# jianzhnie/ScaleRL

Measured on NVIDIA H100. Metric: learner_frames_per_sec, higher is better.
Workload: dtype bf16

## Files before the change

### scalerl_b200/csrc/enc_fused.cuh

```cuda
#pragma once
#include "igemm_tma.cuh"
#include "encoder_problems.cuh"

namespace srl {

constexpr int FF_THREADS = 544;
constexpr int FF_CONV_WARPS = 8;
constexpr int FF_W1_BYTES = 4 * 32 * 128;
constexpr int FF_W2_BYTES = 8 * 64 * 128;
constexpr int FF_U8_BYTES = 28 * 1024;
constexpr int FF_X_BYTES = 19 * 1024;
constexpr int FF_A1_PLANE = 13 * 1024;
constexpr int FF_A1_BYTES = 31 * 1024;
constexpr int FF_OFF_W2 = FF_W1_BYTES;
constexpr int FF_OFF_U8 = FF_OFF_W2 + FF_W2_BYTES;
constexpr int FF_OFF_X = FF_OFF_U8 + 2 * FF_U8_BYTES;
constexpr int FF_XS = 2;
constexpr int FF_OFF_A1 = FF_OFF_X + FF_XS * FF_X_BYTES;
constexpr int FF_OFF_IMG = FF_OFF_A1 + FF_A1_BYTES;
constexpr int FF_OFF_BAR = FF_OFF_IMG + WG_IMG_BYTES;
constexpr int FF_SMEM_BYTES = FF_OFF_BAR + 1024 + 1024;
static_assert(FF_SMEM_BYTES <= 232448, "shared memory budget");
static_assert(FF_OFF_U8 % 1024 == 0 && FF_OFF_X % 1024 == 0 && FF_OFF_A1 % 1024 == 0, "swizzle atoms need 1024-byte aligned tiles");

struct EncFusedParams {
  const uint8_t* obs;
  const float* w1;
  const float* b1;
  const float* w2;
  const float* b2;
  bf16* xs;
  bf16* a1;
  bf16* a2;
  int frames;
  int NFS;
};

SRL_DEVINL void mbar_wait_relaxed(uint64_t* bar, uint32_t parity) {
  uint32_t spins = 0;
  while (!mbar_try_wait(bar, parity)) {
    __nanosleep(32);
    if (++spins > SRL_SPIN_LIMIT) __trap();
  }
}
SRL_DEVINL void bulk_load_1d(void* dst, const void* src, uint32_t bytes, uint64_t* bar) {
  asm volatile("cp.async.bulk.shared::cluster.global.mbarrier::complete_tx::bytes [%0], [%1], %2, [%3];"
               ::"r"(smem_u32(dst)), "l"(src), "r"(bytes), "r"(smem_u32(bar)) : "memory");
}

__global__ void __launch_bounds__(FF_THREADS, 1) enc_fused_fwd_kernel(const EncFusedParams p) {
  extern __shared__ uint8_t smem_raw[];
  uint8_t* smem = reinterpret_cast<uint8_t*>((reinterpret_cast<uintptr_t>(smem_raw) + 1023) & ~uintptr_t(1023));
  uint8_t* sW1 = smem;
  uint8_t* sW2 = smem + FF_OFF_W2;
  uint8_t* sU8 = smem + FF_OFF_U8;
  uint8_t* sX = smem + FF_OFF_X;
  uint8_t* sA1 = smem + FF_OFF_A1;
  uint64_t* bars = reinterpret_cast<uint64_t*>(smem + FF_OFF_BAR);
  uint64_t* u8_full = bars;
  uint64_t* u8_empty = bars + 2;
  uint64_t* x_full = bars + 4;
  uint64_t* x_empty = bars + 7;
  uint64_t* a1_full = bars + 18;
  uint64_t* a1_empty = bars + 19;
  float* img = reinterpret_cast<float*>(smem + FF_OFF_IMG);
  const int tid = threadIdx.x, warp = tid >> 5, lane = tid & 31;
  const int nmine = p.frames > (int)blockIdx.x ? (p.frames - (int)blockIdx.x + (int)gridDim.x - 1) / (int)gridDim.x : 0;

  float* s_b1 = reinterpret_cast<float*>(smem + FF_OFF_BAR + 256);
  float* s_b2 = s_b1 + 32;
  if (tid < 32) s_b1[tid] = __ldg(p.b1 + tid);
  else if (tid < 96) s_b2[tid - 32] = __ldg(p.b2 + tid - 32);
  if (warp == 16 && lane == 0) {
    for (int i = 0; i < 2; ++i) { mbar_init(&u8_full[i], 1); mbar_init(&u8_empty[i], FF_CONV_WARPS); }
    for (int i = 0; i < FF_XS; ++i) { mbar_init(&x_full[i], FF_CONV_WARPS); mbar_init(&x_empty[i], 4); }
    mbar_init(a1_full, 4); mbar_init(a1_empty, 4);
    mbar_fence_init();
  }
  for (int i = tid; i < (FF_A1_BYTES - 2 * FF_A1_PLANE) / 16; i += FF_THREADS)
    reinterpret_cast<uint4*>(sA1 + 2 * FF_A1_PLANE)[i] = make_uint4(0, 0, 0, 0);
  pdl_wait(54);
// ... 26 lines not shown
          const int co = q >> 7, c = (q >> 2) & 31, kh = q & 3;
          const float w[4] = {v[u].x, v[u].y, v[u].z, v[u].w};
#pragma unroll
          for (int kw = 0; kw < 4; ++kw) {
            const int j = kh * 2 + (kw >> 1), k = (kw & 1) * 32 + c;
            *reinterpret_cast<__nv_bfloat16*>(sW2 + j * 8192 + swz128(co, k >> 3) + (k & 7) * 2) = __float2bfloat16_rn(w[kw]);
          }
        }
      }
    }
  }
  fence_proxy_async_smem();
  __syncthreads();

  if (warp == 16) {
    if (lane == 0) {
      for (int it = 0; it < nmine; ++it) {
        const int f = blockIdx.x + it * gridDim.x, ub = it & 1;
        mbar_wait(&u8_empty[ub], ((it >> 1) & 1) ^ 1);
        mbar_arrive_expect_tx(&u8_full[ub], 28224);
        bulk_load_1d(sU8 + ub * FF_U8_BYTES, p.obs + (size_t)f * 28224, 28224, &u8_full[ub]);
      }
    }
  } else if (warp >= 8) {
    const int t = tid - 256, gp = t & 7, rb = t >> 3;
    const int src_g = (gp >> 1) * 7056 + (gp & 1) * 168;
    for (int it = 0; it < nmine; ++it) {
      const int f = blockIdx.x + it * gridDim.x, ub = it & 1;
      mbar_wait_relaxed(&u8_full[ub], (it >> 1) & 1);
      const uint8_t* u8 = sU8 + ub * FF_U8_BYTES + src_g;
      bf16* xs_f = p.xs + (size_t)f * 441 * 64 + gp * 8;
      for (int j = 0; j < 4; ++j) {
        const int n = 4 * it + j, s = n % FF_XS;
        uint32_t w0[5], w1[5];
        int Qs[5];
        {
          int Q = j * 128 + rb, Y = Q / 21, X = Q - Y * 21;
#pragma unroll
          for (int k = 0; k < 5; ++k) {
            Qs[k] = Q;
            if (rb + 32 * k < 150 && Q < 441) {
              w0[k] = *reinterpret_cast<const uint32_t*>(u8 + Y * 336 + 4 * X);
              w1[k] = *reinterpret_cast<const uint32_t*>(u8 + Y * 336 + 84 + 4 * X);
            }
            Q += 32; X += 11; Y += 1;
            if (X >= 21) { X -= 21; Y += 1; }
          }
        }
        mbar_wait(&x_empty[s], ((n / FF_XS) & 1) ^ 1);
        uint8_t* x = sX + s * FF_X_BYTES;
#pragma unroll
        for (int k = 0; k < 5; ++k) {
          const int row = rb + 32 * k;
          if (row < 150) {
            uint4 v = make_uint4(0u, 0u, 0u, 0u);
            if (Qs[k] < 441) {
              v = u8x8_to_bf16x8(w0[k], w1[k]);
              if (row < 128) *reinterpret_cast<uint4*>(xs_f + (size_t)Qs[k] * 64) = v;
            }
            *reinterpret_cast<uint4*>(x + swz128(row, gp)) = v;
          }
        }
        fence_proxy_async_smem();
        __syncwarp();
        if (lane == 0) mbar_arrive(&x_full[s]);
      }
      __syncwarp();
      if (lane == 0) mbar_arrive(&u8_empty[ub]);
    }
  } else if (warp < 4) {
    const uint64_t w1d = make_smem_desc(smem_u32(sW1), 16, 1024);
    for (int it = 0; it < nmine; ++it) {
      const int f = blockIdx.x + it * gridDim.x;
      for (int j = 0; j < 4; ++j) {
        const int n = 4 * it + j, s = n % FF_XS;
        mbar_wait(&x_full[s], (n / FF_XS) & 1);
        const uint64_t xd = make_smem_desc(smem_u32(sX + s * FF_X_BYTES), 16, 1024);
        float acc[2][16];
        wg_fence();
#pragma unroll
        for (int tap = 0; tap < 4; ++tap)
#pragma unroll
          for (int k = 0; k < 4; ++k)
            wg_mma128<32, 0, 0>(acc, xd + (uint64_t)(((tap >> 1) * 21 + (tap & 1)) * 8 + k * 2), 64 * 128 / 16, w1d + (uint64_t)(tap * 256 + k * 2),
                                (tap | k) != 0);
        wg_commit();
        wg_wait_all();
        wg_fence_regs(acc[0]); wg_fence_regs(acc[1]);
        __syncwarp();
        if (lane == 0) mbar_arrive(&x_empty[s]);
        float r0[16], r1[16];
        wg_acc_row16<32, true>(acc, 0, img, tid, 2, r0);
        wg_acc_row16<32, true>(acc, 1, img, tid, 2, r1);
        if (j == 0) mbar_wait_relaxed(a1_empty, (it & 1) ^ 1);
        const int Q = j * 128 + tid, oh = Q / 21, ow = Q - oh * 21;
// ... 72 lines not shown
```

### scalerl_b200/csrc/encoder.cu

```cuda
#include "encoder_problems.cuh"
#include "tma_problems.cuh"
#include "res_problems.cuh"
#include "enc_fused.cuh"
#include "kernels.h"
#include <stdio.h>
#include <stdlib.h>

namespace srl {

constexpr int PACK_BLOCKS_FK = 256, PACK_BLOCKS_FD = 256, PACK_BLOCKS_CONV = 288;
SRL_DEVINL void pack_store(bf16* __restrict__ out, bf16* __restrict__ out_lo, int64_t i, float v) {
  const bf16 hi = __float2bfloat16_rn(v);
  out[i] = hi;
  if (out_lo) out_lo[i] = __float2bfloat16_rn(v - __bfloat162float(hi));
}
SRL_DEVINL void pack_store2(bf16* __restrict__ out, bf16* __restrict__ out_lo, int64_t i, float v0, float v1) {
  const bf16 h0 = __float2bfloat16_rn(v0), h1 = __float2bfloat16_rn(v1);
  *reinterpret_cast<uint32_t*>(out + i) = pack_bf16x2(v0, v1);
  if (out_lo) *reinterpret_cast<uint32_t*>(out_lo + i) = pack_bf16x2(v0 - __bfloat162float(h0), v1 - __bfloat162float(h1));
}
__global__ void __launch_bounds__(256) pack_weights_kernel(ParamPtrs p, bf16* __restrict__ out, bf16* __restrict__ out_lo, int skip_w1k) {
  pdl_wait(2);
  __shared__ __align__(16) float tile[64 * 99];
  const int t = threadIdx.x, b = blockIdx.x;
// ... 281 lines not shown
  if (t >= w) return;
  float s = 0.f;
  for (int c = 0; c < n; ++c) s += stage[c * w + t];
  if (bias) db[t] += s;
  else g[(size_t)(co0 + (t & 7)) * (L::ROW_GROUPS * L::NR) + L::NR * rg + (t >> 3)] = L::FRAMES_U8 ? s * (1.0f / 255.0f) : s;
}

template <class L>
static cudaError_t launch_wgrad_reduce(const float* part, int n, float* g, float* db, cudaStream_t st) {
  static PerDeviceOnce once;
  SRL_TRY(ensure_max_dynamic_smem(once, conv_wgrad_reduce_kernel<L>, WG_PART_CTAS * L::NR * 32));
  static const int greatest = [] { int lo = 0, hi = 0; return cudaDeviceGetStreamPriorityRange(&lo, &hi) == cudaSuccess ? hi : 0; }();
  cudaLaunchConfig_t cfg = {};
  cfg.gridDim = dim3(L::ROW_GROUPS * (L::CO / 8) + 1); cfg.blockDim = dim3(L::NR * 8); cfg.dynamicSmemBytes = (size_t)n * L::NR * 32; cfg.stream = st;
  cudaLaunchAttribute attr[1];
  attr[0].id = cudaLaunchAttributePriority;
  attr[0].val.priority = greatest;
  cfg.attrs = attr; cfg.numAttrs = 1;
  return cudaLaunchKernelEx(&cfg, conv_wgrad_reduce_kernel<L>, part, n, g, db);
}

cudaError_t encoder_forward(const uint8_t* obs, int frames, const ParamPtrs& p, const EncoderBuffers& buf, const TmaMaps& maps, int mode,
                            const StepStreams& S, bool fused_front) {
  if (frames <= 0) return cudaSuccess;
  if ((mode != 0 && mode != 1) || !maps.valid) return cudaErrorInvalidValue;
  const int sp = mode;
  if (sp && !buf.lo.wpack) return cudaErrorInvalidValue;
  const cudaStream_t st = S.main;
  if (fused_front && !sp && (reinterpret_cast<uintptr_t>(obs) & 15) == 0) {
    EncFusedParams q{obs, p.w1, p.b1, p.w2, p.b2, buf.xs, buf.hi.a1, buf.hi.a2, frames, buf.NF};
    S.b(PS_ENC_FUSED); SRL_TRY(enc_fused_fwd_launch(q, kPersistentCtas, st)); S.e(PS_ENC_FUSED);
    SRL_TRY(S.join(LANE_PACK));
  } else {
  S.b(PS_S2D); SRL_TRY(launch_s2d(obs, frames, buf.xs, st, p.w1, buf.hi.wpack + WPack::W1K, sp ? buf.lo.wpack + WPack::W1K : nullptr)); S.e(PS_S2D);
  { RConv1Fwd::Params q{maps.xs_w, maps.hi.w1k, maps.lo.w1k, p.b1, buf.hi.a1, buf.lo.a1, frames, buf.NF};
    S.b(PS_CONV1_FWD); SRL_TRY(res_fwd_launch<RConv1Fwd>(q, cdiv(frames * 441, 128), kPersistentCtas, st, sp)); S.e(PS_CONV1_FWD); }
  SRL_TRY(S.join(LANE_PACK));
  { RConv2Fwd::Params q{maps.hi.a1p0_w, maps.hi.a1p1_w, maps.hi.w2k, maps.lo.a1p0_w, maps.lo.a1p1_w, maps.lo.w2k, p.b2, buf.hi.a2, buf.lo.a2, frames};
    S.b(PS_CONV2_FWD); SRL_TRY(res_fwd_launch<RConv2Fwd>(q, cdiv(frames * 100, 128), kPersistentCtas, st, sp)); S.e(PS_CONV2_FWD); }
  }
  { RConv3Fwd::Params q{maps.hi.a2_w, maps.hi.w3k, maps.lo.a2_w, maps.lo.w3k, p.b3, buf.hi.a3, buf.lo.a3, frames};
    S.b(PS_CONV3_FWD); SRL_TRY(res_fwd_launch<RConv3Fwd>(q, cdiv(frames * 81, 128), kPersistentCtas, st, sp)); S.e(PS_CONV3_FWD); }
  { TFcFwd::Params q{maps.hi.a3m128, maps.hi.wfk, maps.lo.a3m128, maps.lo.wfk, buf.hpart, frames};
    static_assert(TFcFwd::SPLITS == FC_SPLITS, "split count");
    S.b(PS_FC_FWD);
    if (sp) SRL_TRY((igemm_tma_launch<TFcFwd, 1>(q, dim3(cdiv(frames, 128), 8 * FC_SPLITS), st)));
    else SRL_TRY((igemm_tma_launch<TFcFwd, 0>(q, dim3(cdiv(frames, 128), 8 * FC_SPLITS), st)));
    S.e(PS_FC_FWD); }
  return cudaSuccess;
}

cudaError_t encoder_backward(int frames, const EncoderBuffers& buf, const ParamPtrs& g, const TmaMaps& maps, int mode,
                             const StepStreams& S, BwdParts parts, bool a3t_done) {
  if (frames <= 0) return cudaSuccess;
  if ((mode != 0 && mode != 1) || !maps.valid) return cudaErrorInvalidValue;
  const int sp = mode;
  if (sp && !buf.lo.wpack) return cudaErrorInvalidValue;
  const bool do_fc = parts & BWD_FC, do_conv = parts & BWD_CONV;
  const cudaStream_t st = S.main, s1 = S.lane(LANE_FC_WGRAD), s2 = S.lane(LANE_CONV3_WGRAD), s3 = S.lane(LANE_CONV2_WGRAD);
  if (do_fc) {
    SRL_TRY(S.fork(LANE_FC_WGRAD));
    { const bool native = !sp && buf.a3t != nullptr;
      S.b(PS_FC_WGRAD);
      if (native) {
        if (!a3t_done) SRL_TRY(launch_a3_transpose(buf.hi.a3, buf.a3t, frames, s1));
        TFcWgradN::Params q{maps.hi.dhm64, maps.a3tm64, g.wf, g.bf, frames};
        SRL_TRY((igemm_tma_launch<TFcWgradN, 0>(q, dim3(1, 4 * (TFcWgradN::NCT + 1)), s1)));
      } else {
        TFcWgrad::Params q{maps.hi.dhm64, maps.hi.a3m64, maps.lo.dhm64, maps.lo.a3m64, g.wf, g.bf, frames};
// ... 43 lines not shown
```

### scalerl_b200/csrc/encoder_problems.cuh

```cuda
#pragma once
#include "common.cuh"

namespace srl {

typedef __nv_bfloat16 bf16;

SRL_DEVINL uint4 ldg16(const void* p) { return __ldg(reinterpret_cast<const uint4*>(p)); }

SRL_DEVINL uint4 u8x8_to_bf16x8(uint32_t w0, uint32_t w1) {
  float f[8];
  f[0] = __uint_as_float(__byte_perm(w0, 0x4B000000u, 0x7540)) - 8388608.f;
  f[1] = __uint_as_float(__byte_perm(w0, 0x4B000000u, 0x7541)) - 8388608.f;
  f[2] = __uint_as_float(__byte_perm(w0, 0x4B000000u, 0x7542)) - 8388608.f;
  f[3] = __uint_as_float(__byte_perm(w0, 0x4B000000u, 0x7543)) - 8388608.f;
  f[4] = __uint_as_float(__byte_perm(w1, 0x4B000000u, 0x7540)) - 8388608.f;
  f[5] = __uint_as_float(__byte_perm(w1, 0x4B000000u, 0x7541)) - 8388608.f;
  f[6] = __uint_as_float(__byte_perm(w1, 0x4B000000u, 0x7542)) - 8388608.f;
  f[7] = __uint_as_float(__byte_perm(w1, 0x4B000000u, 0x7543)) - 8388608.f;
  return make_uint4(pack_bf16x2(f[0], f[1]), pack_bf16x2(f[2], f[3]), pack_bf16x2(f[4], f[5]), pack_bf16x2(f[6], f[7]));
}

SRL_DEVINL void store_bf16x16(bf16* dst, const float (&v)[16]) {
  uint4 a = make_uint4(pack_bf16x2(v[0], v[1]), pack_bf16x2(v[2], v[3]), pack_bf16x2(v[4], v[5]), pack_bf16x2(v[6], v[7]));
  uint4 b = make_uint4(pack_bf16x2(v[8], v[9]), pack_bf16x2(v[10], v[11]), pack_bf16x2(v[12], v[13]), pack_bf16x2(v[14], v[15]));
  reinterpret_cast<uint4*>(dst)[0] = a;
  reinterpret_cast<uint4*>(dst)[1] = b;
}
SRL_DEVINL void relu_mask16(const bf16* mask, float (&v)[16]) {
  uint4 a = ldg16(mask), b = ldg16(mask + 8);
  const uint32_t w[8] = {a.x, a.y, a.z, a.w, b.x, b.y, b.z, b.w};
#pragma unroll
  for (int i = 0; i < 8; ++i) {
    if (!(bf16_lo(w[i]) > 0.f)) v[2 * i] = 0.f;
    if (!(bf16_hi(w[i]) > 0.f)) v[2 * i + 1] = 0.f;
  }
}

SRL_DEVINL void relu_mask16_pre(const uint4 (&m)[2], float (&v)[16]) {
  const uint32_t w[8] = {m[0].x, m[0].y, m[0].z, m[0].w, m[1].x, m[1].y, m[1].z, m[1].w};
#pragma unroll
  for (int i = 0; i < 8; ++i) {
    if (!(bf16_lo(w[i]) > 0.f)) v[2 * i] = 0.f;
    if (!(bf16_hi(w[i]) > 0.f)) v[2 * i + 1] = 0.f;
  }
}
SRL_DEVINL void ld_mask16(const bf16* mask, uint4 (&m)[2]) { m[0] = ldg16(mask); m[1] = ldg16(mask + 8); }
SRL_DEVINL uint32_t relu_mask_bf16x2(uint32_t x, uint32_t m) {
  return (bf16_lo(m) > 0.f ? x & 0xFFFFu : 0u) | (bf16_hi(m) > 0.f ? x & 0xFFFF0000u : 0u);
}

}
```

### scalerl_b200/csrc/igemm_res.cuh

```cuda
#pragma once
#include "igemm_tma.cuh"

namespace srl {

constexpr int RES_THREADS = 384;
constexpr int RES_PRODUCER_REGS = 40, RES_CONSUMER_REGS = 232;
constexpr int RES_MAX_TAPS = 10;


template <int N, int ROWB, class F>
SRL_DEVINL void wg_acc_stage_bf16(const float (&d)[2][N / 2], uint8_t* buf, int wt, int bar, F f) {
  static_assert(ROWB % 16 == 0 && ROWB >= 2 * N, "16-byte aligned rows that hold N bf16");
  const int w = wt >> 5, l = wt & 31;
  named_bar(bar, 128);
#pragma unroll
  for (int h = 0; h < 2; ++h)
#pragma unroll
    for (int i = 0; i < N / 2; i += 2) {
      const int row = 64 * h + 16 * w + (l >> 2) + 8 * ((i >> 1) & 1), col = 8 * (i >> 2) + 2 * (l & 3);
      *reinterpret_cast<uint32_t*>(buf + row * ROWB + col * 2) = pack_bf16x2(f(col, d[h][i]), f(col + 1, d[h][i + 1]));
    }
  named_bar(bar, 128);
}
template <class P, int SPLIT>
struct ResFwdCfg {
  static constexpr int ALO = (SPLIT && P::A_LO) ? 1 : 0;
  static constexpr int WIN_BYTES = ((P::WROWS * 128 + 1023) / 1024) * 1024;
  static constexpr int IN_HI_BYTES = P::NWIN * WIN_BYTES;
  static constexpr int IN_BYTES = IN_HI_BYTES * (1 + ALO);
  static constexpr int W_HI_BYTES = P::NT * P::BN * 128;
  static constexpr int W_BYTES = W_HI_BYTES * (1 + SPLIT);
  static constexpr bool TILE_EPI = P::TILE_ROWB > 0 && !SPLIT;
  static constexpr int TILE_IMG_BYTES = 128 * P::TILE_ROWB > WG_IMG_BYTES ? 128 * P::TILE_ROWB : WG_IMG_BYTES;
  static constexpr bool IMG1 = !TILE_EPI && W_BYTES + IN_BYTES + 2 * WG_IMG_BYTES + 1024 + 256 > 232448;
  static constexpr int IMG_BYTES = TILE_EPI ? TILE_IMG_BYTES : IMG1 ? WG_IMG_BYTES / 2 : WG_IMG_BYTES;
  static constexpr int FIT = fit_stages(SPLIT ? P::SPLIT_STAGES : P::STAGES, W_BYTES + 2 * IMG_BYTES + 1024 + 256, IN_BYTES);
  static constexpr int STAGES = FIT > 1 ? FIT & ~1 : 1;
  static constexpr int SMEM_BYTES = W_BYTES + STAGES * IN_BYTES + 2 * IMG_BYTES + 1024 + 256;
  static_assert(SMEM_BYTES <= 232448, "shared memory budget (227 KB)");
  static_assert(W_BYTES % 1024 == 0, "weight block alignment");
  static_assert(P::BN == 32 || P::BN == 64 || P::BN == 128, "MMA N");
};

template <class P, int SPLIT>
__global__ void __launch_bounds__(RES_THREADS, 1) res_fwd_kernel(const __grid_constant__ typename P::Params p) {
  using C = ResFwdCfg<P, SPLIT>;
  constexpr int STAGES = C::STAGES;
  extern __shared__ uint8_t smem_raw[];
  uint8_t* smem = reinterpret_cast<uint8_t*>((reinterpret_cast<uintptr_t>(smem_raw) + 1023) & ~uintptr_t(1023));
  uint8_t* sW = smem;
  uint8_t* sIn = smem + C::W_BYTES;
  float* img = reinterpret_cast<float*>(sIn + STAGES * C::IN_BYTES);
  uint64_t* bars = reinterpret_cast<uint64_t*>(sIn + STAGES * C::IN_BYTES + 2 * C::IMG_BYTES);
  uint64_t* in_full = bars;
  uint64_t* in_empty = bars + STAGES;
  uint64_t* w_full = bars + 2 * STAGES;
  const int tid = threadIdx.x, warp = tid >> 5;
  const int ntiles = P::num_tiles(p);

  if (warp == 8 && (tid & 31) == 0) {
    for (int s = 0; s < STAGES; ++s) { mbar_init(&in_full[s], 1); mbar_init(&in_empty[s], 4); }
    mbar_init(w_full, 1);
    mbar_fence_init();
    P::prefetch(p);
  }
  __syncthreads();

  if (warp >= 8) {
    reg_release<RES_PRODUCER_REGS>();
    if (warp != 8) return;
    const uint32_t leader = elect_one_sync();
    auto load_weights = [&]() {
      mbar_arrive_expect_tx(w_full, C::W_BYTES);
      for (int j = 0; j < P::NT; ++j) tma_load_2d(sW + j * P::BN * 128, &p.w, w_full, j * 64, 0);
      if constexpr (SPLIT)
        for (int j = 0; j < P::NT; ++j) tma_load_2d(sW + C::W_HI_BYTES + j * P::BN * 128, &p.w_lo, w_full, j * 64, 0);
    };
    if (leader && !P::W_AFTER_WAIT) load_weights();
    __syncwarp();
    pdl_wait();
    if (leader) pdl_launch();
    if (leader && P::W_AFTER_WAIT) load_weights();
    __syncwarp();
    int it = 0;
    for (int t = blockIdx.x; t < ntiles; t += gridDim.x, ++it) {
      const int s = it % STAGES;
      mbar_wait(&in_empty[s], ((it / STAGES) & 1) ^ 1);
      if (leader) {
        mbar_arrive_expect_tx(&in_full[s], P::NWIN * P::WROWS * 128 * (1 + C::ALO));
        P::load_windows(p, t, sIn + s * C::IN_BYTES, C::WIN_BYTES, &in_full[s], false);
        if constexpr (C::ALO) P::load_windows(p, t, sIn + s * C::IN_BYTES + C::IN_HI_BYTES, C::WIN_BYTES, &in_full[s], true);
      }
      __syncwarp();
    }
  } else {
    reg_claim<RES_CONSUMER_REGS>();
    pdl_wait(P::KID);
    const int g = warp >> 2, wt = tid & 127;
    float* my_img = img + g * (C::IMG_BYTES / 4);
    constexpr uint32_t A_HI = 64 * 128 / 16;
    mbar_wait(w_full, 0);
    const uint64_t wd = make_smem_desc(smem_u32(sW), 16, 1024);
    int it = 0;
    for (int t = blockIdx.x; t < ntiles; t += gridDim.x, ++it) {
      if (STAGES > 1 ? (it & 1) != g : g != 0) continue;
      const int s = it % STAGES;
      uint4 pre[P::BN / 16][2];
      if constexpr (C::TILE_EPI) P::prefetch_tile(p, t, wt, pre);
      else {
#pragma unroll
        for (int c = 0; c < P::BN / 16; ++c) P::prefetch16(p, t, wt, c * 16, pre[c]);
      }
      float acc[2][P::BN / 2];
      mbar_wait(&in_full[s], (it / STAGES) & 1);
      const uint64_t ind = make_smem_desc(smem_u32(sIn + s * C::IN_BYTES), 16, 1024);
      wg_fence();
#pragma unroll
      for (int j = 0; j < P::NT; ++j) {
        const uint64_t ad = ind + (uint64_t)((P::tap_win(j) * C::WIN_BYTES + P::tap_shift(j) * 128) / 16);
        const uint64_t bd = wd + (uint64_t)(j * P::BN * 128 / 16);
#pragma unroll
        for (int k = 0; k < 4; ++k) {
          wg_mma128<P::BN, 0, 0>(acc, ad + 2 * k, A_HI, bd + 2 * k, (j | k) != 0);
          if constexpr (SPLIT)
            wg_mma128<P::BN, 0, 0>(acc, ad + 2 * k, A_HI, bd + (uint64_t)(C::W_HI_BYTES / 16 + 2 * k), 1);
          if constexpr (C::ALO)
            wg_mma128<P::BN, 0, 0>(acc, ad + (uint64_t)(C::IN_HI_BYTES / 16 + 2 * k), A_HI, bd + 2 * k, 1);
        }
      }
// ... 279 lines not shown
```

### scalerl_b200/csrc/igemm_tma.cuh

```cuda
#pragma once
#include <cuda.h>
#include "common.cuh"
#include "kernels.h"

namespace srl {

SRL_DEVINL void tma_prefetch_desc(const CUtensorMap* m) {
  asm volatile("prefetch.tensormap [%0];" ::"l"(reinterpret_cast<uint64_t>(m)) : "memory");
}
SRL_DEVINL void tma_load_2d(void* dst, const CUtensorMap* m, uint64_t* bar, int c0, int c1) {
  asm volatile("cp.async.bulk.tensor.2d.shared::cluster.global.mbarrier::complete_tx::bytes [%0], [%1, {%3, %4}], [%2];"
               ::"r"(smem_u32(dst)), "l"(reinterpret_cast<uint64_t>(m)), "r"(smem_u32(bar)), "r"(c0), "r"(c1) : "memory");
}
SRL_DEVINL void tma_load_3d(void* dst, const CUtensorMap* m, uint64_t* bar, int c0, int c1, int c2) {
  asm volatile("cp.async.bulk.tensor.3d.shared::cluster.global.mbarrier::complete_tx::bytes [%0], [%1, {%3, %4, %5}], [%2];"
               ::"r"(smem_u32(dst)), "l"(reinterpret_cast<uint64_t>(m)), "r"(smem_u32(bar)), "r"(c0), "r"(c1), "r"(c2) : "memory");
}
SRL_DEVINL void tma_load_4d(void* dst, const CUtensorMap* m, uint64_t* bar, int c0, int c1, int c2, int c3) {
  asm volatile("cp.async.bulk.tensor.4d.shared::cluster.global.mbarrier::complete_tx::bytes [%0], [%1, {%3, %4, %5, %6}], [%2];"
               ::"r"(smem_u32(dst)), "l"(reinterpret_cast<uint64_t>(m)), "r"(smem_u32(bar)), "r"(c0), "r"(c1), "r"(c2), "r"(c3)
               : "memory");
}
SRL_DEVINL void tma_load_5d(void* dst, const CUtensorMap* m, uint64_t* bar, int c0, int c1, int c2, int c3, int c4) {
  asm volatile("cp.async.bulk.tensor.5d.shared::cluster.global.mbarrier::complete_tx::bytes [%0], [%1, {%3, %4, %5, %6, %7}], [%2];"
               ::"r"(smem_u32(dst)), "l"(reinterpret_cast<uint64_t>(m)), "r"(smem_u32(bar)), "r"(c0), "r"(c1), "r"(c2), "r"(c3), "r"(c4)
               : "memory");
}

constexpr int IGT_THREADS = 288;

template <class P, int SPLIT = 0>
struct TmaCfg {
  static constexpr int KROWS = P::A_MN ? P::KROWS : 64;
  static constexpr int A_BYTES = P::A_MN ? 2 * KROWS * 128 : 128 * 128;
  static constexpr int B_BLOCKS = (P::BN + 63) / 64;
  static constexpr int B_BYTES = P::B_MN ? B_BLOCKS * KROWS * 128 : P::BN * 128;
  static constexpr int HALF_BYTES = A_BYTES + B_BYTES;
  static constexpr int STAGE_BYTES = HALF_BYTES * (1 + SPLIT);
  static constexpr int NB = P::BN / 2;
  static constexpr int STAGES = fit_stages(P::STAGES, 2 * WG_IMG_BYTES + 1024 + 256, STAGE_BYTES);
  static constexpr int SMEM_BYTES = STAGES * STAGE_BYTES + 2 * WG_IMG_BYTES + 1024 + 256;
  static_assert(SMEM_BYTES <= 232448, "shared memory budget (227 KB)");
  static_assert(NB == 32 || NB == 64 || NB == 128, "MMA N per warpgroup");
  static constexpr int MMAS = P::A_MN ? KROWS / 16 : 4;
  static constexpr bool TILE_EPI = P::TILE_ROWB > 0 && !SPLIT;
// ... 149 lines not shown
```

### scalerl_b200/csrc/res_problems.cuh

```cuda
#pragma once
#include "igemm_res.cuh"
#include "encoder_problems.cuh"

namespace srl {

template <int SPLIT>
SRL_DEVINL void store_act16(bf16* hi, bf16* lo, size_t elem_off, const float (&v)[16]) {
  store_bf16x16(hi + elem_off, v);
  if constexpr (SPLIT) {
    float r[16];
#pragma unroll
    for (int j = 0; j < 16; ++j) r[j] = v[j] - __bfloat162float(__float2bfloat16_rn(v[j]));
    store_bf16x16(lo + elem_off, r);
  }
}

struct RConv1Fwd {
  static constexpr int KID = 11;
  static constexpr int BN = 32, NT = 4, NWIN = 1, WROWS = 128 + 22, STAGES = 4, SPLIT_STAGES = 4;
  static constexpr bool A_LO = false;
  struct Params { SRL_TMAP in0; SRL_TMAP w; SRL_TMAP w_lo; const float* bias; bf16* out; bf16* out_lo; int NF; int NFS; };
  static constexpr bool W_AFTER_WAIT = true;
  SRL_DEVINL static void prefetch(const Params& p) { tma_prefetch_desc(&p.in0); tma_prefetch_desc(&p.w); }
  SRL_DEVINL static int num_tiles(const Params& p) { return (p.NF * 441 + 127) >> 7; }
  SRL_DEVINL static constexpr int tap_win(int) { return 0; }
  SRL_DEVINL static constexpr int tap_shift(int j) { return (j >> 1) * 21 + (j & 1); }
  SRL_DEVINL static void load_windows(const Params& p, int t, uint8_t* dst, int, uint64_t* bar, bool) { tma_load_2d(dst, &p.in0, bar, 0, t * 128); }
  SRL_DEVINL static void prefetch16(const Params&, int, int, int, uint4 (&)[2]) {}
  static constexpr int TILE_ROWB = 80;
  SRL_DEVINL static void prefetch_tile(const Params&, int, int, uint4 (&)[BN / 16][2]) {}
  SRL_DEVINL static void epilogue_tile(const Params& p, int t, int wt, const float (&acc)[2][BN / 2], uint8_t* img, int bar,
                                       const uint4 (&)[BN / 16][2]) {
    wg_acc_stage_bf16<BN, TILE_ROWB>(acc, img, wt, bar, [&](int c, float v) { return fmaxf(fmaf(v, 1.0f / 255.0f, __ldg(p.bias + c)), 0.f); });
#pragma unroll
    for (int s = 0; s < 4; ++s) {
      const int e = s * 128 + wt, q = e >> 2, k = e & 3;
      const int Q = t * 128 + q, n = Q / 441, r = Q - n * 441, oh = r / 21, ow = r - oh * 21;
      if (n >= p.NF || oh >= 20 || ow >= 20) continue;
      const size_t prow = (size_t)(oh & 1) * p.NFS * 100 + (size_t)n * 100 + (oh >> 1) * 10 + (ow >> 1);
      *reinterpret_cast<uint4*>(p.out + prow * 64 + (ow & 1) * 32 + k * 8) = *reinterpret_cast<const uint4*>(img + q * TILE_ROWB + k * 16);
    }
  }
  template <int SPLIT>
  SRL_DEVINL static void epilogue16(const Params& p, int t, int row, int c0, float (&v)[16], const uint4 (&)[2]) {
    const int Q = t * 128 + row, n = Q / 441, r = Q - n * 441, oh = r / 21, ow = r - oh * 21;
    if (n >= p.NF || oh >= 20 || ow >= 20) return;
#pragma unroll
    for (int j = 0; j < 16; ++j) v[j] = fmaxf(fmaf(v[j], 1.0f / 255.0f, __ldg(p.bias + c0 + j)), 0.f);
    const size_t prow = (size_t)(oh & 1) * p.NFS * 100 + (size_t)n * 100 + (oh >> 1) * 10 + (ow >> 1);
    store_act16<SPLIT>(p.out, p.out_lo, prow * 64 + (ow & 1) * 32 + c0, v);
  }
};

struct RConv2Fwd {
  static constexpr int KID = 12;
  static constexpr bool W_AFTER_WAIT = false;
  static constexpr int BN = 64, NT = 8, NWIN = 2, WROWS = 128 + 11, STAGES = 3, SPLIT_STAGES = 1;
  static constexpr bool A_LO = true;
  struct Params { SRL_TMAP in0; SRL_TMAP in1; SRL_TMAP w; SRL_TMAP in0_lo; SRL_TMAP in1_lo; SRL_TMAP w_lo; const float* bias; bf16* out; bf16* out_lo; int NF; };
  SRL_DEVINL static void prefetch(const Params& p) { tma_prefetch_desc(&p.in0); tma_prefetch_desc(&p.in1); tma_prefetch_desc(&p.w); }
  SRL_DEVINL static int num_tiles(const Params& p) { return (p.NF * 100 + 127) >> 7; }
  SRL_DEVINL static constexpr int tap_win(int j) { return (j >> 1) & 1; }
  SRL_DEVINL static constexpr int tap_shift(int j) { return (j >> 2) * 10 + (j & 1); }
  SRL_DEVINL static void load_windows(const Params& p, int t, uint8_t* dst, int win_bytes, uint64_t* bar, bool lo) {
    tma_load_2d(dst, lo ? &p.in0_lo : &p.in0, bar, 0, t * 128);
    tma_load_2d(dst + win_bytes, lo ? &p.in1_lo : &p.in1, bar, 0, t * 128);
  }
  SRL_DEVINL static void prefetch16(const Params&, int, int, int, uint4 (&)[2]) {}
  static constexpr int TILE_ROWB = 144;
  SRL_DEVINL static void prefetch_tile(const Params&, int, int, uint4 (&)[BN / 16][2]) {}
  SRL_DEVINL static void epilogue_tile(const Params& p, int t, int wt, const float (&acc)[2][BN / 2], uint8_t* img, int bar,
                                       const uint4 (&)[BN / 16][2]) {
    wg_acc_stage_bf16<BN, TILE_ROWB>(acc, img, wt, bar, [&](int c, float v) { return fmaxf(v + __ldg(p.bias + c), 0.f); });
#pragma unroll
    for (int s = 0; s < 8; ++s) {
      const int e = s * 128 + wt, q = e >> 3, k = e & 7;
      const int Q = t * 128 + q, n = Q / 100, r = Q - n * 100, oh = r / 10, ow = r - oh * 10;
      if (n >= p.NF || oh >= 9 || ow >= 9) continue;
      *reinterpret_cast<uint4*>(p.out + ((size_t)n * 81 + oh * 9 + ow) * 64 + k * 8) = *reinterpret_cast<const uint4*>(img + q * TILE_ROWB + k * 16);
    }
  }
  template <int SPLIT>
  SRL_DEVINL static void epilogue16(const Params& p, int t, int row, int c0, float (&v)[16], const uint4 (&)[2]) {
    const int Q = t * 128 + row, n = Q / 100, r = Q - n * 100, oh = r / 10, ow = r - oh * 10;
    if (n >= p.NF || oh >= 9 || ow >= 9) return;
#pragma unroll
    for (int j = 0; j < 16; ++j) v[j] = fmaxf(v[j] + __ldg(p.bias + c0 + j), 0.f);
    store_act16<SPLIT>(p.out, p.out_lo, ((size_t)n * 81 + oh * 9 + ow) * 64 + c0, v);
  }
};

struct RConv3Fwd {
  static constexpr int KID = 13;
  static constexpr bool W_AFTER_WAIT = false;
  static constexpr int BN = 64, NT = 9, NWIN = 1, WROWS = 128 + 20, STAGES = 4, SPLIT_STAGES = 2;
  static constexpr bool A_LO = true;
  struct Params { SRL_TMAP in0; SRL_TMAP w; SRL_TMAP in0_lo; SRL_TMAP w_lo; const float* bias; bf16* out; bf16* out_lo; int NF; };
  SRL_DEVINL static void prefetch(const Params& p) { tma_prefetch_desc(&p.in0); tma_prefetch_desc(&p.w); }
  SRL_DEVINL static int num_tiles(const Params& p) { return (p.NF * 81 + 127) >> 7; }
  SRL_DEVINL static constexpr int tap_win(int) { return 0; }
  SRL_DEVINL static constexpr int tap_shift(int j) { return (j / 3) * 9 + j % 3; }
  SRL_DEVINL static void load_windows(const Params& p, int t, uint8_t* dst, int, uint64_t* bar, bool lo) { tma_load_2d(dst, lo ? &p.in0_lo : &p.in0, bar, 0, t * 128); }
  SRL_DEVINL static void prefetch16(const Params&, int, int, int, uint4 (&)[2]) {}
  static constexpr int TILE_ROWB = 144;
  SRL_DEVINL static void prefetch_tile(const Params&, int, int, uint4 (&)[BN / 16][2]) {}
  SRL_DEVINL static void epilogue_tile(const Params& p, int t, int wt, const float (&acc)[2][BN / 2], uint8_t* img, int bar,
                                       const uint4 (&)[BN / 16][2]) {
    wg_acc_stage_bf16<BN, TILE_ROWB>(acc, img, wt, bar, [&](int c, float v) { return fmaxf(v + __ldg(p.bias + c), 0.f); });
#pragma unroll
    for (int s = 0; s < 8; ++s) {
      const int e = s * 128 + wt, q = e >> 3, k = e & 7;
      const int Q = t * 128 + q, n = Q / 81, r = Q - n * 81, oh = r / 9, ow = r - oh * 9;
      if (n >= p.NF || oh >= 7 || ow >= 7) continue;
      *reinterpret_cast<uint4*>(p.out + ((size_t)n * 49 + oh * 7 + ow) * 64 + k * 8) = *reinterpret_cast<const uint4*>(img + q * TILE_ROWB + k * 16);
    }
  }
  template <int SPLIT>
  SRL_DEVINL static void epilogue16(const Params& p, int t, int row, int c0, float (&v)[16], const uint4 (&)[2]) {
    const int Q = t * 128 + row, n = Q / 81, r = Q - n * 81, oh = r / 9, ow = r - oh * 9;
    if (n >= p.NF || oh >= 7 || ow >= 7) return;
#pragma unroll
    for (int j = 0; j < 16; ++j) v[j] = fmaxf(v[j] + __ldg(p.bias + c0 + j), 0.f);
    store_act16<SPLIT>(p.out, p.out_lo, ((size_t)n * 49 + oh * 7 + ow) * 64 + c0, v);
  }
};

struct RConv3Dgrad {
  static constexpr int KID = 14;
  static constexpr bool W_AFTER_WAIT = false;
  static constexpr int BN = 64, NT = 9, NWIN = 1, WROWS = 128 + 20, STAGES = 4, SPLIT_STAGES = 2;
  static constexpr bool A_LO = true;
  struct Params { SRL_TMAP in0; SRL_TMAP w; SRL_TMAP in0_lo; SRL_TMAP w_lo; const bf16* act; bf16* dx; bf16* dx_lo; int NB; };
  SRL_DEVINL static void prefetch(const Params& p) { tma_prefetch_desc(&p.in0); tma_prefetch_desc(&p.w); }
  SRL_DEVINL static int num_tiles(const Params& p) { return (p.NB * 81 + 127) >> 7; }
  SRL_DEVINL static constexpr int tap_win(int) { return 0; }
  SRL_DEVINL static constexpr int tap_shift(int j) { return 20 - ((j / 3) * 9 + j % 3); }
  SRL_DEVINL static void load_windows(const Params& p, int t, uint8_t* dst, int, uint64_t* bar, bool lo) { tma_load_2d(dst, lo ? &p.in0_lo : &p.in0, bar, 0, t * 128 - 20); }
  SRL_DEVINL static void prefetch16(const Params& p, int t, int row, int c0, uint4 (&m)[2]) {
    const int Q = t * 128 + row;
    if (Q < p.NB * 81) ld_mask16(p.act + (size_t)Q * 64 + c0, m);
  }
  static constexpr int TILE_ROWB = 144;
  SRL_DEVINL static void prefetch_tile(const Params& p, int t, int wt, uint4 (&m)[BN / 16][2]) {
#pragma unroll
    for (int s = 0; s < 8; ++s) {
      const int e = s * 128 + wt, Q = t * 128 + (e >> 3);
      if (Q < p.NB * 81) m[s >> 1][s & 1] = ldg16(p.act + (size_t)Q * 64 + (e & 7) * 8);
    }
  }
  SRL_DEVINL static void epilogue_tile(const Params& p, int t, int wt, const float (&acc)[2][BN / 2], uint8_t* img, int bar,
                                       const uint4 (&m)[BN / 16][2]) {
    wg_acc_stage_bf16<BN, TILE_ROWB>(acc, img, wt, bar, [](int, float v) { return v; });
#pragma unroll
    for (int s = 0; s < 8; ++s) {
      const int e = s * 128 + wt, q = e >> 3, k = e & 7;
      const int Q = t * 128 + q, n = Q / 81, r = Q - n * 81, ih = r / 9, iw = r - ih * 9;
      if (n >= p.NB) continue;
      const uint4 x = *reinterpret_cast<const uint4*>(img + q * TILE_ROWB + k * 16), mk = m[s >> 1][s & 1];
      *reinterpret_cast<uint4*>(p.dx + ((size_t)n * 100 + ih * 10 + iw) * 64 + k * 8) =
          make_uint4(relu_mask_bf16x2(x.x, mk.x), relu_mask_bf16x2(x.y, mk.y), relu_mask_bf16x2(x.z, mk.z), relu_mask_bf16x2(x.w, mk.w));
    }
  }
  template <int SPLIT>
  SRL_DEVINL static void epilogue16(const Params& p, int t, int row, int c0, float (&v)[16], const uint4 (&m)[2]) {
    const int Q = t * 128 + row, n = Q / 81, r = Q - n * 81, ih = r / 9, iw = r - ih * 9;
    if (n >= p.NB) return;
    relu_mask16_pre(m, v);
    store_act16<SPLIT>(p.dx, p.dx_lo, ((size_t)n * 100 + ih * 10 + iw) * 64 + c0, v);
  }
};

struct RConv2Dgrad {
  static constexpr int KID = 15;
  static constexpr bool W_AFTER_WAIT = false;
  static constexpr int BN = 128, NT = 4, NWIN = 1, WROWS = 128 + 11, STAGES = 3, SPLIT_STAGES = 2;
  static constexpr bool A_LO = true;
  struct Params { SRL_TMAP in0; SRL_TMAP w; SRL_TMAP in0_lo; SRL_TMAP w_lo; const bf16* act; bf16* dx; bf16* dx_lo; int NB; int NF; };
  SRL_DEVINL static void prefetch(const Params& p) { tma_prefetch_desc(&p.in0); tma_prefetch_desc(&p.w); }
  SRL_DEVINL static int num_tiles(const Params& p) { return (p.NB * 100 + 127) >> 7; }
  SRL_DEVINL static constexpr int tap_win(int) { return 0; }
  SRL_DEVINL static constexpr int tap_shift(int j) { return 11 - ((j >> 1) * 10 + (j & 1)); }
  SRL_DEVINL static void load_windows(const Params& p, int t, uint8_t* dst, int, uint64_t* bar, bool lo) { tma_load_2d(dst, lo ? &p.in0_lo : &p.in0, bar, 0, t * 128 - 11); }
  SRL_DEVINL static void prefetch16(const Params& p, int t, int row, int c0, uint4 (&m)[2]) {
    const int Q = t * 128 + row, cls = c0 >> 5, c = c0 & 31;
    if (Q < p.NB * 100) ld_mask16(p.act + ((size_t)(cls >> 1) * p.NF * 100 + Q) * 64 + (cls & 1) * 32 + c, m);
  }
  static constexpr int TILE_ROWB = 272;
  SRL_DEVINL static void prefetch_tile(const Params& p, int t, int wt, uint4 (&m)[BN / 16][2]) {
#pragma unroll
    for (int s = 0; s < 16; ++s) {
      const int e = s * 128 + wt, ph = e >> 10, Q = t * 128 + ((e >> 3) & 127);
      if (Q < p.NB * 100) m[s >> 1][s & 1] = ldg16(p.act + ((size_t)ph * p.NF * 100 + Q) * 64 + (e & 7) * 8);
    }
  }
  SRL_DEVINL static void epilogue_tile(const Params& p, int t, int wt, const float (&acc)[2][BN / 2], uint8_t* img, int bar,
                                       const uint4 (&m)[BN / 16][2]) {
    wg_acc_stage_bf16<BN, TILE_ROWB>(acc, img, wt, bar, [](int, float v) { return v; });
#pragma unroll
    for (int s = 0; s < 16; ++s) {
      const int e = s * 128 + wt, ph = e >> 10, q = (e >> 3) & 127, k = e & 7;
      const int Q = t * 128 + q, n = Q / 100, r = Q - n * 100, i = r / 10, j = r - i * 10;
      if (n >= p.NB) continue;
      const uint4 x = *reinterpret_cast<const uint4*>(img + q * TILE_ROWB + ph * 128 + k * 16), mk = m[s >> 1][s & 1];
      *reinterpret_cast<uint4*>(p.dx + ((size_t)n * 441 + (2 * i + ph) * 21 + 2 * j) * 32 + k * 8) =
          make_uint4(relu_mask_bf16x2(x.x, mk.x), relu_mask_bf16x2(x.y, mk.y), relu_mask_bf16x2(x.z, mk.z), relu_mask_bf16x2(x.w, mk.w));
    }
  }
// ... 58 lines not shown
```

Baseline: 2.692 million.

## Fuse uint8 space-to-depth conversion into conv1 forward producer warps

When the fused encoder front is not used, conv1 forward in bf16 mode now reads raw uint8 observations via bulk copies, and converter warps 9-11 turn them into swizzled bf16 tiles in shared memory. This replaces the separate s2d kernel launch, which now runs with zero frames. The xs buffer is still written from the converters for backward use. It adds extra shared memory stages, barriers and a rebalance of producer and consumer registers, which may reduce pipeline stages.

```diff
diff --git a/scalerl_b200/csrc/enc_fused.cuh b/scalerl_b200/csrc/enc_fused.cuh
--- a/scalerl_b200/csrc/enc_fused.cuh
+++ b/scalerl_b200/csrc/enc_fused.cuh
@@ -43,10 +43,6 @@
     if (++spins > SRL_SPIN_LIMIT) __trap();
   }
 }
-SRL_DEVINL void bulk_load_1d(void* dst, const void* src, uint32_t bytes, uint64_t* bar) {
-  asm volatile("cp.async.bulk.shared::cluster.global.mbarrier::complete_tx::bytes [%0], [%1], %2, [%3];"
-               ::"r"(smem_u32(dst)), "l"(src), "r"(bytes), "r"(smem_u32(bar)) : "memory");
-}
 
 __global__ void __launch_bounds__(FF_THREADS, 1) enc_fused_fwd_kernel(const EncFusedParams p) {
   extern __shared__ uint8_t smem_raw[];
@@ -139,35 +135,12 @@
       bf16* xs_f = p.xs + (size_t)f * 441 * 64 + gp * 8;
       for (int j = 0; j < 4; ++j) {
         const int n = 4 * it + j, s = n % FF_XS;
-        uint32_t w0[5], w1[5];
-        int Qs[5];
-        {
-          int Q = j * 128 + rb, Y = Q / 21, X = Q - Y * 21;
-#pragma unroll
-          for (int k = 0; k < 5; ++k) {
-            Qs[k] = Q;
-            if (rb + 32 * k < 150 && Q < 441) {
-              w0[k] = *reinterpret_cast<const uint32_t*>(u8 + Y * 336 + 4 * X);
-              w1[k] = *reinterpret_cast<const uint32_t*>(u8 + Y * 336 + 84 + 4 * X);
-            }
-            Q += 32; X += 11; Y += 1;
-            if (X >= 21) { X -= 21; Y += 1; }
-          }
-        }
+        S2dWindow<32> win;
+        win.load(u8, rb, j * 128, 441);
         mbar_wait(&x_empty[s], ((n / FF_XS) & 1) ^ 1);
-        uint8_t* x = sX + s * FF_X_BYTES;
-#pragma unroll
-        for (int k = 0; k < 5; ++k) {
-          const int row = rb + 32 * k;
-          if (row < 150) {
-            uint4 v = make_uint4(0u, 0u, 0u, 0u);
-            if (Qs[k] < 441) {
-              v = u8x8_to_bf16x8(w0[k], w1[k]);
-              if (row < 128) *reinterpret_cast<uint4*>(xs_f + (size_t)Qs[k] * 64) = v;
-            }
-            *reinterpret_cast<uint4*>(x + swz128(row, gp)) = v;
-          }
-        }
+        win.store(sX + s * FF_X_BYTES, gp, rb, [&](int row, uint4 v) {
+          if (row < 128) *reinterpret_cast<uint4*>(xs_f + (size_t)(j * 128 + row) * 64) = v;
+        });
         fence_proxy_async_smem();
         __syncwarp();
         if (lane == 0) mbar_arrive(&x_full[s]);
diff --git a/scalerl_b200/csrc/encoder.cu b/scalerl_b200/csrc/encoder.cu
--- a/scalerl_b200/csrc/encoder.cu
+++ b/scalerl_b200/csrc/encoder.cu
@@ -337,9 +337,15 @@
     S.b(PS_ENC_FUSED); SRL_TRY(enc_fused_fwd_launch(q, kPersistentCtas, st)); S.e(PS_ENC_FUSED);
     SRL_TRY(S.join(LANE_PACK));
   } else {
-  S.b(PS_S2D); SRL_TRY(launch_s2d(obs, frames, buf.xs, st, p.w1, buf.hi.wpack + WPack::W1K, sp ? buf.lo.wpack + WPack::W1K : nullptr)); S.e(PS_S2D);
+  const bool u8_feed = !sp && (reinterpret_cast<uintptr_t>(obs) & 15) == 0;
+  S.b(PS_S2D);
+  SRL_TRY(launch_s2d(obs, u8_feed ? 0 : frames, buf.xs, st, p.w1, buf.hi.wpack + WPack::W1K, sp ? buf.lo.wpack + WPack::W1K : nullptr));
+  S.e(PS_S2D);
   { RConv1Fwd::Params q{maps.xs_w, maps.hi.w1k, maps.lo.w1k, p.b1, buf.hi.a1, buf.lo.a1, frames, buf.NF};
-    S.b(PS_CONV1_FWD); SRL_TRY(res_fwd_launch<RConv1Fwd>(q, cdiv(frames * 441, 128), kPersistentCtas, st, sp)); S.e(PS_CONV1_FWD); }
+    S.b(PS_CONV1_FWD);
+    if (u8_feed) SRL_TRY((res_fwd_launch_t<RConv1Fwd::FromFrames, 0>(RConv1Fwd::FromFrames::Params{q, obs, buf.xs}, cdiv(frames * 441, 128), kPersistentCtas, st)));
+    else SRL_TRY(res_fwd_launch<RConv1Fwd>(q, cdiv(frames * 441, 128), kPersistentCtas, st, sp));
+    S.e(PS_CONV1_FWD); }
   SRL_TRY(S.join(LANE_PACK));
   { RConv2Fwd::Params q{maps.hi.a1p0_w, maps.hi.a1p1_w, maps.hi.w2k, maps.lo.a1p0_w, maps.lo.a1p1_w, maps.lo.w2k, p.b2, buf.hi.a2, buf.lo.a2, frames};
     S.b(PS_CONV2_FWD); SRL_TRY(res_fwd_launch<RConv2Fwd>(q, cdiv(frames * 100, 128), kPersistentCtas, st, sp)); S.e(PS_CONV2_FWD); }
diff --git a/scalerl_b200/csrc/encoder_problems.cuh b/scalerl_b200/csrc/encoder_problems.cuh
--- a/scalerl_b200/csrc/encoder_problems.cuh
+++ b/scalerl_b200/csrc/encoder_problems.cuh
@@ -19,6 +19,42 @@
   f[7] = __uint_as_float(__byte_perm(w1, 0x4B000000u, 0x7543)) - 8388608.f;
   return make_uint4(pack_bf16x2(f[0], f[1]), pack_bf16x2(f[2], f[3]), pack_bf16x2(f[4], f[5]), pack_bf16x2(f[6], f[7]));
 }
+
+template <int SLOTS>
+struct S2dWindow {
+  static constexpr int ROWS = 150, K = (ROWS + SLOTS - 1) / SLOTS;
+  uint32_t w0[K], w1[K], valid = 0;
+  SRL_DEVINL void load(const uint8_t* img, int rb, int q0, int qend) {
+    const uint32_t base = smem_u32(img);
+    int q = q0 + rb, Y = q / 21, X = q - Y * 21;
+#pragma unroll
+    for (int k = 0; k < K; ++k) {
+      w0[k] = 0u; w1[k] = 0u;
+      if (rb + SLOTS * k < ROWS && q < qend) {
+        const uint32_t a = base + Y * 336 + 4 * X;
+        asm volatile("ld.shared.b32 %0, [%1];" : "=r"(w0[k]) : "r"(a) : "memory");
+        asm volatile("ld.shared.b32 %0, [%1];" : "=r"(w1[k]) : "r"(a + 84) : "memory");
+        valid |= 1u << k;
+      }
+      q += SLOTS; X += SLOTS % 21; Y += SLOTS / 21;
+      if (X >= 21) { X -= 21; Y += 1; }
+    }
+  }
+  template <class F>
+  SRL_DEVINL void store(uint8_t* win, int gp, int rb, F&& f) const {
+    const uint32_t base = smem_u32(win);
+#pragma unroll
+    for (int k = 0; k < K; ++k) {
+      const int row = rb + SLOTS * k;
+      if (SLOTS * (k + 1) <= ROWS || row < ROWS) {
+        const uint4 v = u8x8_to_bf16x8(w0[k], w1[k]);
+        if ((valid >> k) & 1) f(row, v);
+        asm volatile("st.shared.v4.b32 [%0], {%1, %2, %3, %4};" ::"r"(base + swz128(row, gp)), "r"(v.x), "r"(v.y), "r"(v.z), "r"(v.w)
+                     : "memory");
+      }
+    }
+  }
+};
 
 SRL_DEVINL void store_bf16x16(bf16* dst, const float (&v)[16]) {
   uint4 a = make_uint4(pack_bf16x2(v[0], v[1]), pack_bf16x2(v[2], v[3]), pack_bf16x2(v[4], v[5]), pack_bf16x2(v[6], v[7]));
diff --git a/scalerl_b200/csrc/igemm_res.cuh b/scalerl_b200/csrc/igemm_res.cuh
--- a/scalerl_b200/csrc/igemm_res.cuh
+++ b/scalerl_b200/csrc/igemm_res.cuh
@@ -1,5 +1,6 @@
 #pragma once
 #include "igemm_tma.cuh"
+#include "encoder_problems.cuh"
 
 namespace srl {
 
@@ -28,19 +29,48 @@
   static constexpr int WIN_BYTES = ((P::WROWS * 128 + 1023) / 1024) * 1024;
   static constexpr int IN_HI_BYTES = P::NWIN * WIN_BYTES;
   static constexpr int IN_BYTES = IN_HI_BYTES * (1 + ALO);
+  static constexpr bool U8 = P::U8_BYTES > 0;
+  static constexpr int U8_BYTES = P::U8_BYTES;
+  static_assert(!U8 || (!SPLIT && P::NWIN == 1), "u8-fed windows: bf16 mode, one window");
+  static constexpr int PRODUCER_REGS = U8 ? 72 : RES_PRODUCER_REGS, CONSUMER_REGS = U8 ? 216 : RES_CONSUMER_REGS;
+  static_assert(PRODUCER_REGS + 2 * CONSUMER_REGS <= 3 * (65536 / RES_THREADS & ~7), "register budgets within the launch allocation");
   static constexpr int W_HI_BYTES = P::NT * P::BN * 128;
   static constexpr int W_BYTES = W_HI_BYTES * (1 + SPLIT);
   static constexpr bool TILE_EPI = P::TILE_ROWB > 0 && !SPLIT;
   static constexpr int TILE_IMG_BYTES = 128 * P::TILE_ROWB > WG_IMG_BYTES ? 128 * P::TILE_ROWB : WG_IMG_BYTES;
   static constexpr bool IMG1 = !TILE_EPI && W_BYTES + IN_BYTES + 2 * WG_IMG_BYTES + 1024 + 256 > 232448;
   static constexpr int IMG_BYTES = TILE_EPI ? TILE_IMG_BYTES : IMG1 ? WG_IMG_BYTES / 2 : WG_IMG_BYTES;
-  static constexpr int FIT = fit_stages(SPLIT ? P::SPLIT_STAGES : P::STAGES, W_BYTES + 2 * IMG_BYTES + 1024 + 256, IN_BYTES);
+  static constexpr int FIT = fit_stages(SPLIT ? P::SPLIT_STAGES : P::STAGES, W_BYTES + 2 * IMG_BYTES + 1024 + 256, IN_BYTES + U8_BYTES);
   static constexpr int STAGES = FIT > 1 ? FIT & ~1 : 1;
-  static constexpr int SMEM_BYTES = W_BYTES + STAGES * IN_BYTES + 2 * IMG_BYTES + 1024 + 256;
+  static constexpr int SMEM_BYTES = W_BYTES + STAGES * (IN_BYTES + U8_BYTES) + 2 * IMG_BYTES + 1024 + 256;
   static_assert(SMEM_BYTES <= 232448, "shared memory budget (227 KB)");
   static_assert(W_BYTES % 1024 == 0, "weight block alignment");
   static_assert(P::BN == 32 || P::BN == 64 || P::BN == 128, "MMA N");
 };
+
+template <class P, class C>
+SRL_DEVINL void res_u8_converters(const typename P::Params& p, uint8_t* sIn, uint8_t* sU8, uint64_t* in_full, uint64_t* in_empty,
+                                  uint64_t* u8_full, uint64_t* u8_empty, int tid) {
+  constexpr int STAGES = C::STAGES;
+  static_assert(P::CONV_SLOTS == 12, "warps 9-11");
+  const int ct = tid - 288, gp = ct & 7, rb = ct >> 3;
+  const int ntiles = P::num_tiles(p), qend = p.NF * 441;
+  const int plane = (gp >> 1) * P::U8_PLANE + (gp & 1) * 168;
+  int it = 0;
+  for (int t = blockIdx.x; t < ntiles; t += gridDim.x, ++it) {
+    const int s = it % STAGES, q0 = t * 128, r0 = q0 / 21;
+    const uint32_t ph = (it / STAGES) & 1;
+    S2dWindow<P::CONV_SLOTS> w;
+    mbar_wait(&u8_full[s], ph);
+    w.load(sU8 + s * C::U8_BYTES + plane, rb, q0 - r0 * 21, qend - r0 * 21);
+    mbar_wait(&in_empty[s], ph ^ 1);
+    bf16* xs = p.xs + (size_t)q0 * 64 + gp * 8;
+    w.store(sIn + s * C::IN_BYTES, gp, rb, [&](int row, uint4 v) { if (row < 128) *reinterpret_cast<uint4*>(xs + (size_t)row * 64) = v; });
+    fence_proxy_async_smem();
+    __syncwarp();
+    if ((tid & 31) == 0) { mbar_arrive(&u8_empty[s]); mbar_arrive(&in_full[s]); }
+  }
+}
 
 template <class P, int SPLIT>
 __global__ void __launch_bounds__(RES_THREADS, 1) res_fwd_kernel(const __grid_constant__ typename P::Params p) {
@@ -51,15 +81,20 @@
   uint8_t* sW = smem;
   uint8_t* sIn = smem + C::W_BYTES;
   float* img = reinterpret_cast<float*>(sIn + STAGES * C::IN_BYTES);
-  uint64_t* bars = reinterpret_cast<uint64_t*>(sIn + STAGES * C::IN_BYTES + 2 * C::IMG_BYTES);
+  uint8_t* sU8 = sIn + STAGES * C::IN_BYTES + 2 * C::IMG_BYTES;
+  uint64_t* bars = reinterpret_cast<uint64_t*>(sU8 + STAGES * C::U8_BYTES);
   uint64_t* in_full = bars;
   uint64_t* in_empty = bars + STAGES;
   uint64_t* w_full = bars + 2 * STAGES;
+  uint64_t* u8_full = bars + 2 * STAGES + 1;
+  uint64_t* u8_empty = bars + 3 * STAGES + 1;
   const int tid = threadIdx.x, warp = tid >> 5;
   const int ntiles = P::num_tiles(p);
 
   if (warp == 8 && (tid & 31) == 0) {
-    for (int s = 0; s < STAGES; ++s) { mbar_init(&in_full[s], 1); mbar_init(&in_empty[s], 4); }
+    for (int s = 0; s < STAGES; ++s) { mbar_init(&in_full[s], C::U8 ? 3 : 1); mbar_init(&in_empty[s], 4); }
+    if constexpr (C::U8)
+      for (int s = 0; s < STAGES; ++s) { mbar_init(&u8_full[s], 1); mbar_init(&u8_empty[s], 3); }
     mbar_init(w_full, 1);
     mbar_fence_init();
     P::prefetch(p);
@@ -67,8 +102,10 @@
   __syncthreads();
 
   if (warp >= 8) {
-    reg_release<RES_PRODUCER_REGS>();
-    if (warp != 8) return;
+    reg_release<C::PRODUCER_REGS>();
+    if constexpr (C::U8) {
+      if (warp != 8) { res_u8_converters<P, C>(p, sIn, sU8, in_full, in_empty, u8_full, u8_empty, tid); return; }
+    } else if (warp != 8) return;
     const uint32_t leader = elect_one_sync();
     auto load_weights = [&]() {
       mbar_arrive_expect_tx(w_full, C::W_BYTES);
@@ -85,16 +122,21 @@
     int it = 0;
     for (int t = blockIdx.x; t < ntiles; t += gridDim.x, ++it) {
       const int s = it % STAGES;
-      mbar_wait(&in_empty[s], ((it / STAGES) & 1) ^ 1);
-      if (leader) {
-        mbar_arrive_expect_tx(&in_full[s], P::NWIN * P::WROWS * 128 * (1 + C::ALO));
-        P::load_windows(p, t, sIn + s * C::IN_BYTES, C::WIN_BYTES, &in_full[s], false);
-        if constexpr (C::ALO) P::load_windows(p, t, sIn + s * C::IN_BYTES + C::IN_HI_BYTES, C::WIN_BYTES, &in_full[s], true);
+      if constexpr (C::U8) {
+        mbar_wait(&u8_empty[s], ((it / STAGES) & 1) ^ 1);
+        if (leader) P::load_u8(p, t, sU8 + s * C::U8_BYTES, &u8_full[s]);
+      } else {
+        mbar_wait(&in_empty[s], ((it / STAGES) & 1) ^ 1);
+        if (leader) {
+          mbar_arrive_expect_tx(&in_full[s], P::NWIN * P::WROWS * 128 * (1 + C::ALO));
+          P::load_windows(p, t, sIn + s * C::IN_BYTES, C::WIN_BYTES, &in_full[s], false);
+          if constexpr (C::ALO) P::load_windows(p, t, sIn + s * C::IN_BYTES + C::IN_HI_BYTES, C::WIN_BYTES, &in_full[s], true);
+        }
       }
       __syncwarp();
     }
   } else {
-    reg_claim<RES_CONSUMER_REGS>();
+    reg_claim<C::CONSUMER_REGS>();
     pdl_wait(P::KID);
     const int g = warp >> 2, wt = tid & 127;
     float* my_img = img + g * (C::IMG_BYTES / 4);
diff --git a/scalerl_b200/csrc/igemm_tma.cuh b/scalerl_b200/csrc/igemm_tma.cuh
--- a/scalerl_b200/csrc/igemm_tma.cuh
+++ b/scalerl_b200/csrc/igemm_tma.cuh
@@ -11,6 +11,10 @@
 SRL_DEVINL void tma_load_2d(void* dst, const CUtensorMap* m, uint64_t* bar, int c0, int c1) {
   asm volatile("cp.async.bulk.tensor.2d.shared::cluster.global.mbarrier::complete_tx::bytes [%0], [%1, {%3, %4}], [%2];"
                ::"r"(smem_u32(dst)), "l"(reinterpret_cast<uint64_t>(m)), "r"(smem_u32(bar)), "r"(c0), "r"(c1) : "memory");
+}
+SRL_DEVINL void bulk_load_1d(void* dst, const void* src, uint32_t bytes, uint64_t* bar) {
+  asm volatile("cp.async.bulk.shared::cluster.global.mbarrier::complete_tx::bytes [%0], [%1], %2, [%3];"
+               ::"r"(smem_u32(dst)), "l"(src), "r"(bytes), "r"(smem_u32(bar)) : "memory");
 }
 SRL_DEVINL void tma_load_3d(void* dst, const CUtensorMap* m, uint64_t* bar, int c0, int c1, int c2) {
   asm volatile("cp.async.bulk.tensor.3d.shared::cluster.global.mbarrier::complete_tx::bytes [%0], [%1, {%3, %4, %5}], [%2];"
diff --git a/scalerl_b200/csrc/res_problems.cuh b/scalerl_b200/csrc/res_problems.cuh
--- a/scalerl_b200/csrc/res_problems.cuh
+++ b/scalerl_b200/csrc/res_problems.cuh
@@ -21,6 +21,8 @@
   static constexpr bool A_LO = false;
   struct Params { SRL_TMAP in0; SRL_TMAP w; SRL_TMAP w_lo; const float* bias; bf16* out; bf16* out_lo; int NF; int NFS; };
   static constexpr bool W_AFTER_WAIT = true;
+  static constexpr int U8_BYTES = 0;
+  struct FromFrames;
   SRL_DEVINL static void prefetch(const Params& p) { tma_prefetch_desc(&p.in0); tma_prefetch_desc(&p.w); }
   SRL_DEVINL static int num_tiles(const Params& p) { return (p.NF * 441 + 127) >> 7; }
   SRL_DEVINL static constexpr int tap_win(int) { return 0; }
@@ -52,9 +54,29 @@
   }
 };
 
+struct RConv1Fwd::FromFrames : RConv1Fwd {
+  static constexpr int SPAN = 9;
+  static constexpr int U8_PLANE = SPAN * 336;
+  static constexpr int U8_BYTES = 4 * U8_PLANE;
+  static constexpr int CONV_SLOTS = 12;
+  struct Params : RConv1Fwd::Params { const uint8_t* obs; bf16* xs; };
+  SRL_DEVINL static void prefetch(const Params& p) { tma_prefetch_desc(&p.w); }
+  SRL_DEVINL static void load_u8(const Params& p, int t, uint8_t* dst, uint64_t* bar) {
+    const int q0 = t * 128, q1 = min(q0 + WROWS, p.NF * 441) - 1, r0 = q0 / 21, r1 = q1 / 21;
+    mbar_arrive_expect_tx(bar, (r1 - r0 + 1) * 4 * 336);
+    for (int ra = r0; ra <= r1;) {
+      const int n = ra / 21, rz = min(r1, n * 21 + 20);
+      const uint8_t* src = p.obs + (size_t)n * 28224 + (ra - n * 21) * 336;
+      for (int c = 0; c < 4; ++c) bulk_load_1d(dst + c * U8_PLANE + (ra - r0) * 336, src + c * 7056, (rz - ra + 1) * 336, bar);
+      ra = rz + 1;
+    }
+  }
+};
+
 struct RConv2Fwd {
   static constexpr int KID = 12;
   static constexpr bool W_AFTER_WAIT = false;
+  static constexpr int U8_BYTES = 0;
   static constexpr int BN = 64, NT = 8, NWIN = 2, WROWS = 128 + 11, STAGES = 3, SPLIT_STAGES = 1;
   static constexpr bool A_LO = true;
   struct Params { SRL_TMAP in0; SRL_TMAP in1; SRL_TMAP w; SRL_TMAP in0_lo; SRL_TMAP in1_lo; SRL_TMAP w_lo; const float* bias; bf16* out; bf16* out_lo; int NF; };
@@ -93,6 +115,7 @@
 struct RConv3Fwd {
   static constexpr int KID = 13;
   static constexpr bool W_AFTER_WAIT = false;
+  static constexpr int U8_BYTES = 0;
   static constexpr int BN = 64, NT = 9, NWIN = 1, WROWS = 128 + 20, STAGES = 4, SPLIT_STAGES = 2;
   static constexpr bool A_LO = true;
   struct Params { SRL_TMAP in0; SRL_TMAP w; SRL_TMAP in0_lo; SRL_TMAP w_lo; const float* bias; bf16* out; bf16* out_lo; int NF; };
@@ -128,6 +151,7 @@
 struct RConv3Dgrad {
   static constexpr int KID = 14;
   static constexpr bool W_AFTER_WAIT = false;
+  static constexpr int U8_BYTES = 0;
   static constexpr int BN = 64, NT = 9, NWIN = 1, WROWS = 128 + 20, STAGES = 4, SPLIT_STAGES = 2;
   static constexpr bool A_LO = true;
   struct Params { SRL_TMAP in0; SRL_TMAP w; SRL_TMAP in0_lo; SRL_TMAP w_lo; const bf16* act; bf16* dx; bf16* dx_lo; int NB; };
@@ -173,6 +197,7 @@
 struct RConv2Dgrad {
   static constexpr int KID = 15;
   static constexpr bool W_AFTER_WAIT = false;
+  static constexpr int U8_BYTES = 0;
   static constexpr int BN = 128, NT = 4, NWIN = 1, WROWS = 128 + 11, STAGES = 3, SPLIT_STAGES = 2;
   static constexpr bool A_LO = true;
   struct Params { SRL_TMAP in0; SRL_TMAP w; SRL_TMAP in0_lo; SRL_TMAP w_lo; const bf16* act; bf16* dx; bf16* dx_lo; int NB; int NF; };
```

Result: faster. 2.839 million (median of 6 runs) (+5.4%).
